# Suyashagarw/StreamOptima

Hardware: AMD Instinct MI355X
Metric: encoded Mpixels/sec at 1080p & 4K, 1/2/4/8 GPUs; PSNR delta vs reference (higher is better)
Workload: dtype u8

## Files before the change

### streamoptima_amd/csrc/so_block.h

```cpp
#pragma once
#include "so_common.h"
#include "so_dct.h"

namespace so {

SO_DEV void wave_sync() {
    __builtin_amdgcn_fence(__ATOMIC_RELEASE, "wavefront");
    __builtin_amdgcn_wave_barrier();
    __builtin_amdgcn_fence(__ATOMIC_ACQUIRE, "wavefront");
}

SO_DEV int scan_index(int n, int i, int j) {
    const int k = i + j;
    const int before = (k < n) ? (k * (k + 1)) / 2 : n * n - ((2 * n - 1 - k) * (2 * n - k)) / 2;
    const int first_i = (k < n) ? 0 : k - n + 1;
    return before + (i - first_i);
}

template <int G>
SO_DEV int group_sum(int v) {
#pragma unroll
    for (int m = G / 2; m >= 1; m >>= 1) v += __shfl_xor(v, m, 64);
    return v;
}

template <int NB>
SO_DEV void fetch_row(const uint8_t* __restrict__ f, int W, int H, int px, int py, bool fast, int* out) {
    if (fast) {
        const uint8_t* p = f + (size_t)py * W + px;
        const uintptr_t a = reinterpret_cast<uintptr_t>(p);
        const uint32_t* q = reinterpret_cast<const uint32_t*>(a & ~(uintptr_t)3);
        const uint32_t sh = (uint32_t)(a & 3);
        uint32_t w[NB / 4 + 1];
#pragma unroll
        for (int k = 0; k <= NB / 4; ++k) w[k] = q[k];
#pragma unroll
        for (int k = 0; k < NB / 4; ++k) {
            uint32_t v = __builtin_amdgcn_alignbyte(w[k + 1], w[k], sh);
            out[4 * k + 0] = v & 255;
            out[4 * k + 1] = (v >> 8) & 255;
            out[4 * k + 2] = (v >> 16) & 255;
            out[4 * k + 3] = v >> 24;
        }
    } else {
#pragma unroll
        for (int k = 0; k < NB; ++k) {
            const int xx = px + k;
            out[k] = (py >= 0 && py < H && xx >= 0 && xx < W) ? f[(size_t)py * W + xx] : 0;
        }
    }
}

template <int NB>
SO_DEV void fetch_row_fme(const uint8_t* __restrict__ planes, size_t pstride, int W, int H, int px, int py, int row,
                          int ext, int lim, int* out) {
    const int W2 = 2 * W - 1, H2 = 2 * H - 1;
    if (0 <= px && px < W2 - NB && 0 <= py && py < H2 - NB) {
        if (0 <= px + ext && px + ext < W2 - lim && 0 <= py + ext && py + ext < H2 - lim) {
            const uint8_t* pl = planes + (size_t)(2 * (py & 1) + (px & 1)) * pstride;
            fetch_row<NB>(pl, W, H, px >> 1, (py >> 1) + row, true, out);
        } else {
#pragma unroll
            for (int k = 0; k < NB; ++k) out[k] = 128;
        }
    } else {
        const int Y = py + row;
#pragma unroll
        for (int k = 0; k < NB; ++k) {
            const int X = px + k;
            out[k] = (Y >= 0 && Y < H2 && X >= 0 && X < W2)
                         ? planes[(size_t)(2 * (Y & 1) + (X & 1)) * pstride + (size_t)(Y >> 1) * W + (X >> 1)]
                         : 0;
        }
    }
}

template <int NB>
SO_DEV void load_cur_row(const uint8_t* __restrict__ f, int W, int x, int y, int* out) {
    const uint8_t* p = f + (size_t)y * W + x;
    if constexpr (NB == 16) {
        uint4 v = *reinterpret_cast<const uint4*>(p);
        uint32_t w[4] = {v.x, v.y, v.z, v.w};
#pragma unroll
        for (int k = 0; k < 16; ++k) out[k] = (w[k >> 2] >> (8 * (k & 3))) & 255;
    } else {
        uint2 v = *reinterpret_cast<const uint2*>(p);
        uint32_t w[2] = {v.x, v.y};
#pragma unroll
        for (int k = 0; k < 8; ++k) out[k] = (w[k >> 2] >> (8 * (k & 3))) & 255;
    }
}

template <int NB>
SO_DEV void store_row_u8(uint8_t* __restrict__ f, int W, int x, int y, const int* v) {
    uint32_t w[NB / 4];
#pragma unroll
    for (int k = 0; k < NB / 4; ++k)
        w[k] = (uint32_t)(v[4 * k] & 255) | ((uint32_t)(v[4 * k + 1] & 255) << 8) |
               ((uint32_t)(v[4 * k + 2] & 255) << 16) | ((uint32_t)(v[4 * k + 3] & 255) << 24);
    uint8_t* p = f + (size_t)y * W + x;
    if constexpr (NB == 16) *reinterpret_cast<uint4*>(p) = make_uint4(w[0], w[1], w[2], w[3]);
    else *reinterpret_cast<uint2*>(p) = make_uint2(w[0], w[1]);
}

template <int NB>
SO_DEV void store_row_i16(int16_t* __restrict__ p, const int* v) {
    uint32_t w[NB / 2];
#pragma unroll
    for (int k = 0; k < NB / 2; ++k) w[k] = (uint32_t)(uint16_t)v[2 * k] | ((uint32_t)(uint16_t)v[2 * k + 1] << 16);
    if constexpr (NB == 16) {
        reinterpret_cast<uint4*>(p)[0] = make_uint4(w[0], w[1], w[2], w[3]);
        reinterpret_cast<uint4*>(p)[1] = make_uint4(w[4], w[5], w[6], w[7]);
    } else {
        reinterpret_cast<uint4*>(p)[0] = make_uint4(w[0], w[1], w[2], w[3]);
    }
}

template <int NB>
SO_DEV void load_row_i16(const int16_t* __restrict__ p, int* v) {
    uint32_t w[NB / 2];
    if constexpr (NB == 16) {
        uint4 a = reinterpret_cast<const uint4*>(p)[0], b = reinterpret_cast<const uint4*>(p)[1];
        w[0] = a.x; w[1] = a.y; w[2] = a.z; w[3] = a.w; w[4] = b.x; w[5] = b.y; w[6] = b.z; w[7] = b.w;
    } else {
        uint4 a = reinterpret_cast<const uint4*>(p)[0];
        w[0] = a.x; w[1] = a.y; w[2] = a.z; w[3] = a.w;
    }
#pragma unroll
    for (int k = 0; k < NB / 2; ++k) {
        v[2 * k] = (int)(int16_t)(w[k] & 0xFFFF);
        v[2 * k + 1] = (int)(int16_t)(w[k] >> 16);
    }
}

template <int N, bool INVERSE, class T, class TWt = typename dct::Rfft<N>::TW>
SO_DEV void xform2d_rows(double* lds, int l, const T* in_row, double* out_row, const TWt& tw = TWt{}) {
    constexpr int P = N + 1;
    double v[N];
    if constexpr (N == 16 && __is_same(T, int)) {
        int* const li = reinterpret_cast<int*>(lds);
#pragma unroll
        for (int c = 0; c < N; ++c) li[l * P + c] = in_row[c];
        wave_sync();
        int x[N];
#pragma unroll
        for (int r = 0; r < N; ++r) x[r] = li[r * P + l];
        wave_sync();
        if constexpr (INVERSE) dct::dct3_16_i(x, v, tw); else dct::dct2_16_i(x, v, tw);
    } else {
#pragma unroll
        for (int c = 0; c < N; ++c) lds[l * P + c] = (double)in_row[c];
        wave_sync();
#pragma unroll
        for (int r = 0; r < N; ++r) v[r] = lds[r * P + l];
        if constexpr (INVERSE) dct::dct3<N>(v, tw); else dct::dct2<N>(v, tw);
    }
#pragma unroll
    for (int r = 0; r < N; ++r) lds[r * P + l] = v[r];
    wave_sync();
#pragma unroll
    for (int c = 0; c < N; ++c) v[c] = lds[l * P + c];
    if constexpr (INVERSE) dct::dct3<N>(v, tw); else dct::dct2<N>(v, tw);
#pragma unroll
    for (int c = 0; c < N; ++c) out_row[c] = v[c];
    wave_sync();
}

template <bool INVERSE, class TWt>
SO_DEV void xform2d_rows_dw(double* lds, int l, const int* in_row, double* out_row, const TWt& tw) {
    constexpr int N = 16, P = N + 1;
    typedef __attribute__((address_space(3))) uint32_t* lds_u32p;
    lds_u32p rowp = (lds_u32p)(reinterpret_cast<uint32_t*>(lds) + l * P);
    lds_u32p colp = (lds_u32p)(reinterpret_cast<uint32_t*>(lds) + l);
    asm volatile("" : "+v"(rowp), "+v"(colp));
    double v[N];
    {
#pragma unroll
        for (int c = 0; c < N; ++c) rowp[c] = (uint32_t)in_row[c];
        wave_sync();
        int x[N];
#pragma unroll
        for (int r = 0; r < N; ++r) x[r] = (int)colp[r * P];
        wave_sync();
        if constexpr (INVERSE) dct::dct3_16_i(x, v, tw); else dct::dct2_16_i(x, v, tw);
    }
    uint32_t lo[N];
#pragma unroll
    for (int r = 0; r < N; ++r) colp[r * P] = (uint32_t)__builtin_bit_cast(uint64_t, v[r]);
    wave_sync();
#pragma unroll
    for (int c = 0; c < N; ++c) lo[c] = rowp[c];
    wave_sync();
#pragma unroll
    for (int r = 0; r < N; ++r) colp[r * P] = (uint32_t)(__builtin_bit_cast(uint64_t, v[r]) >> 32);
    wave_sync();
#pragma unroll
    for (int c = 0; c < N; ++c)
        v[c] = __builtin_bit_cast(double, ((uint64_t)rowp[c] << 32) | (uint64_t)lo[c]);
    if constexpr (INVERSE) dct::dct3<N>(v, tw); else dct::dct2<N>(v, tw);
#pragma unroll
    for (int c = 0; c < N; ++c) out_row[c] = v[c];
    wave_sync();
}

template <bool INVERSE, bool DW, class FT>
SO_DEV void xform2d_fast(double* lds, int l, const int* in_row, double (&v)[16], const FT& ft) {
    constexpr int N = 16, P = N + 1;
    typedef __attribute__((address_space(3))) uint32_t* lds_u32p;
    lds_u32p rowp = (lds_u32p)(reinterpret_cast<uint32_t*>(lds) + l * P);
    lds_u32p colp = (lds_u32p)(reinterpret_cast<uint32_t*>(lds) + l);
    if constexpr (DW) asm volatile("" : "+v"(rowp), "+v"(colp));
    {
#pragma unroll
        for (int c = 0; c < N; ++c) rowp[c] = (uint32_t)in_row[c];
        wave_sync();
        int x[N];
#pragma unroll
        for (int r = 0; r < N; ++r) x[r] = (int)colp[r * P];
        wave_sync();
        if constexpr (INVERSE) {
#pragma unroll
            for (int r = 0; r < N; ++r) v[r] = (double)x[r];
            dct::dct3_16_fast(v, ft);
        } else {
            dct::dct2_16_fast_i(x, v, ft);
        }
    }
    if constexpr (DW) {
        uint32_t lo[N];
#pragma unroll
        for (int r = 0; r < N; ++r) colp[r * P] = (uint32_t)__builtin_bit_cast(uint64_t, v[r]);
        wave_sync();
#pragma unroll
        for (int c = 0; c < N; ++c) lo[c] = rowp[c];
        wave_sync();
#pragma unroll
        for (int r = 0; r < N; ++r) colp[r * P] = (uint32_t)(__builtin_bit_cast(uint64_t, v[r]) >> 32);
        wave_sync();
#pragma unroll
        for (int c = 0; c < N; ++c) v[c] = __builtin_bit_cast(double, ((uint64_t)rowp[c] << 32) | (uint64_t)lo[c]);
    } else {
#pragma unroll
        for (int r = 0; r < N; ++r) lds[r * P + l] = v[r];
        wave_sync();
#pragma unroll
        for (int c = 0; c < N; ++c) v[c] = lds[l * P + c];
    }
    if constexpr (INVERSE) dct::dct3_16_fast(v, ft); else dct::dct2_16_fast(v, ft);
    wave_sync();
}

template <class TWt>
SO_DEV void xform2d_fwd_i_half(double* lds, int l, const int* in_row, double* out_row, const TWt& tw) {
    constexpr int N = 16, PI = N + 1, P = 9;
    const int hl = l >> 3, cl = l & 7;
    double v[N];
    {
        int* const li = reinterpret_cast<int*>(lds);
#pragma unroll
        for (int c = 0; c < N; ++c) li[l * PI + c] = in_row[c];
        wave_sync();
        int x[N];
#pragma unroll
        for (int r = 0; r < N; ++r) x[r] = li[r * PI + l];
        wave_sync();
        dct::dct2_16_i(x, v, tw);
    }
#pragma unroll
    for (int h = 0; h < 2; ++h) {
        if (hl == h) {
#pragma unroll
            for (int r = 0; r < N; ++r) lds[r * P + cl] = v[r];
        }
        wave_sync();
#pragma unroll
        for (int c = 0; c < 8; ++c) out_row[8 * h + c] = lds[l * P + c];
        wave_sync();
    }
    dct::dct2<N>(out_row, tw);
}

template <bool INVERSE, class T>
SO_DEV void xform2d_rows_half(double* lds, int l, const T* in_row, double* out_row) {
    constexpr int N = 16, P = 9;
    const int hl = l >> 3, cl = l & 7;
    double v[N];
#pragma unroll
    for (int h = 0; h < 2; ++h) {
#pragma unroll
        for (int c = 0; c < 8; ++c) lds[l * P + c] = (double)in_row[8 * h + c];
        wave_sync();
        if (hl == h) {
#pragma unroll
            for (int r = 0; r < N; ++r) v[r] = lds[r * P + cl];
        }
        wave_sync();
    }
    if constexpr (INVERSE) dct::dct3<N>(v); else dct::dct2<N>(v);
#pragma unroll
    for (int h = 0; h < 2; ++h) {
        if (hl == h) {
#pragma unroll
            for (int r = 0; r < N; ++r) lds[r * P + cl] = v[r];
        }
        wave_sync();
#pragma unroll
        for (int c = 0; c < 8; ++c) out_row[8 * h + c] = lds[l * P + c];
        wave_sync();
    }
    if constexpr (INVERSE) dct::dct3<N>(out_row); else dct::dct2<N>(out_row);
}

template <bool INVERSE, class T, class TWt = dct::TW8>
SO_DEV void xform2d_sub(double* lds, int l, const T (&in)[2][8], double (&out)[2][8], const TWt& tw = TWt{}) {
    const int j = l >> 2, r0 = l & 3;
    double* s = lds + j * 72;
    if constexpr (__is_same(T, int)) {
        int* const si = reinterpret_cast<int*>(s);
#pragma unroll
        for (int h = 0; h < 2; ++h)
#pragma unroll
            for (int c = 0; c < 8; ++c) si[(r0 + 4 * h) * 9 + c] = in[h][c];
        wave_sync();
        int x[2][8];
#pragma unroll
        for (int h = 0; h < 2; ++h)
#pragma unroll
            for (int r = 0; r < 8; ++r) x[h][r] = si[r * 9 + r0 + 4 * h];
        wave_sync();
#pragma unroll
        for (int h = 0; h < 2; ++h) {
            double v[8];
            if constexpr (INVERSE) dct::dct3_8_i(x[h], v, tw); else dct::dct2_8_i(x[h], v, tw);
#pragma unroll
            for (int r = 0; r < 8; ++r) s[r * 9 + r0 + 4 * h] = v[r];
        }
    } else {
#pragma unroll
        for (int h = 0; h < 2; ++h)
#pragma unroll
            for (int c = 0; c < 8; ++c) s[(r0 + 4 * h) * 9 + c] = (double)in[h][c];
        wave_sync();
#pragma unroll
        for (int h = 0; h < 2; ++h) {
            double v[8];
            const int col = r0 + 4 * h;
#pragma unroll
            for (int r = 0; r < 8; ++r) v[r] = s[r * 9 + col];
            if constexpr (INVERSE) dct::dct3<8>(v, tw); else dct::dct2<8>(v, tw);
#pragma unroll
            for (int r = 0; r < 8; ++r) s[r * 9 + col] = v[r];
        }
    }
    wave_sync();
#pragma unroll
    for (int h = 0; h < 2; ++h) {
        double v[8];
        const int row = r0 + 4 * h;
#pragma unroll
        for (int c = 0; c < 8; ++c) v[c] = s[row * 9 + c];
        if constexpr (INVERSE) dct::dct3<8>(v, tw); else dct::dct2<8>(v, tw);
#pragma unroll
        for (int c = 0; c < 8; ++c) out[h][c] = v[c];
    }
    wave_sync();
}

template <int N>
SO_DEV void quant_row(const int* tc, int row, int qp, int* q) {
#pragma unroll
    for (int c = 0; c < N; ++c) q[c] = quant_rne(tc[c], q_exp(row, c, N, qp));
}

template <int N>
SO_DEV void dequant_row(const int* q, int row, int qp, int* d) {
#pragma unroll
    for (int c = 0; c < N; ++c) d[c] = q[c] * (1 << q_exp(row, c, N, qp));
}

template <int N>
SO_DEV int q_exp_fast(int row, int c, int qp) {
    const int s = row + c - (N - 2);
    return qp + (s < 0 ? 0 : (s > 2 ? 2 : s));
}

template <int N>
SO_DEV void quant_row_d(const double* tcr, int row, int qp, double* qd, int* q) {
#pragma unroll
    for (int c = 0; c < N; ++c) {
        qd[c] = __builtin_rint(__builtin_amdgcn_ldexp(tcr[c], -q_exp_fast<N>(row, c, qp)));
        q[c] = (int)qd[c];
    }
}

template <int N>
SO_DEV void dequant_row_d(const double* qd, int row, int qp, double* dq) {
#pragma unroll
    for (int c = 0; c < N; ++c) dq[c] = __builtin_amdgcn_ldexp(qd[c], q_exp_fast<N>(row, c, qp));
}

template <int N>
SO_DEV void quant_row_i(const int* tc, int row, int qp, int* q) {
#pragma unroll
    for (int c = 0; c < N; ++c)
        q[c] = (int)__builtin_rint(__builtin_amdgcn_ldexp((double)tc[c], -q_exp_fast<N>(row, c, qp)));
}

template <int N>
SO_DEV void dequant_row_i(const int* q, int row, int qp, double* dq) {
#pragma unroll
    for (int c = 0; c < N; ++c) dq[c] = __builtin_amdgcn_ldexp((double)q[c], q_exp_fast<N>(row, c, qp));
}

SO_DEV int quant_rne_i(int tc, int k) {
    const int bias = k > 0 ? ((1 << k) >> 1) - 1 + ((tc >> k) & 1) : 0;
    return (tc + bias) >> k;
}
template <int N>
SO_DEV void quant_row_int(const int* tc, int row, int qp, int* q) {
#pragma unroll
    for (int c = 0; c < N; ++c) q[c] = quant_rne_i(tc[c], q_exp_fast<N>(row, c, qp));
}

template <int N>
SO_DEV void dequant_row_int(const int* q, int row, int qp, int* dq) {
#pragma unroll
    for (int c = 0; c < N; ++c) dq[c] = (int)((uint32_t)q[c] << q_exp_fast<N>(row, c, qp));
}

template <int N>
SO_DEV int block_tokens(uint8_t* flags, int l, const int* q) {
    (void)flags;
    uint32_t m = 0;
#pragma unroll
    for (int c = 0; c < N; ++c) m |= (q[c] != 0 ? 1u : 0u) << c;
    const uint32_t mn = (uint32_t)__builtin_amdgcn_update_dpp(0, (int)m, 0x101, 0xF, 0xF, false);
    uint32_t m0, mlast;
    if constexpr (N == 16) {
        m0 = (uint32_t)__builtin_amdgcn_update_dpp(0, (int)m, 0x150, 0xF, 0xF, false);
        mlast = (uint32_t)__builtin_amdgcn_update_dpp(0, (int)m, 0x150 + N - 1, 0xF, 0xF, false);
    } else {
        const int base = (threadIdx.x & 63) & ~(N - 1);
        m0 = (uint32_t)__shfl((int)m, base, 64);
        mlast = (uint32_t)__shfl((int)m, base + N - 1, 64);
    }
    constexpr uint32_t kInner = ((1u << N) - 1) & ~1u;
    int tr = 0;
    if (l <= N - 2) {
        tr += __builtin_popcount((m ^ (mn << 1)) & kInner);
        tr += (int)((m & 1u) ^ ((m0 >> (l + 1)) & 1u));
    }
    if (l >= 1) tr += (int)(((mlast >> (l - 1)) & 1u) ^ ((m >> (N - 1)) & 1u));
    return group_sum<N>(__builtin_popcount(m) + tr) + 1;
}

SO_DEV int sub_tokens(uint8_t* flags, int l, const int (&q)[2][8]) {
    const int j = l >> 2, r0 = l & 3;
    uint8_t* s = flags + j * 64;
#pragma unroll
    for (int h = 0; h < 2; ++h)
#pragma unroll
        for (int c = 0; c < 8; ++c) s[scan_index(8, r0 + 4 * h, c)] = q[h][c] != 0;
    wave_sync();
    int nnz = 0, tr = 0;
    const int base = r0 * 16;
    int prev = s[base == 0 ? 0 : base - 1];
#pragma unroll
    for (int k = 0; k < 16; ++k) {
        const int f = s[base + k];
        nnz += f;
        tr += (f != prev);
        prev = f;
    }
    wave_sync();
    return group_sum<16>(nnz + tr) + 4;
}

SO_DEV int sub_tokens_reg(int l, const int (&q)[2][8]) {
    const int r0 = l & 3;
    uint32_t m0 = 0, m1 = 0;
#pragma unroll
    for (int c = 0; c < 8; ++c) {
        m0 |= (q[0][c] != 0 ? 1u : 0u) << c;
        m1 |= (q[1][c] != 0 ? 1u : 0u) << c;
    }
    uint32_t lo = m0 << (8 * r0), hi = m1 << (8 * r0);
    lo |= (uint32_t)__builtin_amdgcn_update_dpp(0, (int)lo, 0xB1, 0xF, 0xF, false);
    hi |= (uint32_t)__builtin_amdgcn_update_dpp(0, (int)hi, 0xB1, 0xF, 0xF, false);
    lo |= (uint32_t)__builtin_amdgcn_update_dpp(0, (int)lo, 0x4E, 0xF, 0xF, false);
    hi |= (uint32_t)__builtin_amdgcn_update_dpp(0, (int)hi, 0x4E, 0xF, 0xF, false);
    const uint32_t n0 = r0 < 3 ? (lo >> (8 * r0 + 8)) & 255u : hi & 255u;
    const uint32_t n1 = r0 < 3 ? (hi >> (8 * r0 + 8)) & 255u : 0u;
    const uint32_t M0 = lo & 255u, M7 = hi >> 24;
    int tr = __builtin_popcount((m0 ^ (n0 << 1)) & 0xFEu) + (int)((m0 & 1u) ^ ((M0 >> (r0 + 1)) & 1u)) +
             (int)(((M7 >> (r0 + 3)) & 1u) ^ (m1 >> 7));
    if (r0 < 3) tr += __builtin_popcount((m1 ^ (n1 << 1)) & 0xFEu) + (int)((m1 & 1u) ^ ((M0 >> (r0 + 5)) & 1u));
    if (r0 >= 1) tr += (int)(((M7 >> (r0 - 1)) & 1u) ^ (m0 >> 7));
    return group_sum<16>(__builtin_popcount(m0) + __builtin_popcount(m1) + tr) + 4;
}

SO_DEV double rd_cost(double lam, int bits, double mae) {
    const double lb = lam * (double)bits;
    return lb + mae;
}

}
```

### streamoptima_amd/csrc/so_me.hip

```cpp
#include <stdlib.h>
#include <string.h>

#include <array>
#include <cstring>
#include <map>
#include <mutex>
#include <type_traits>
#include <utility>

#include "so_block.h"
#include "so_common.h"
#include "so_dpp.h"
#include "so_run.h"

namespace so {

SO_DEV uint64_t me_key(uint32_t sad, uint32_t l1, uint32_t ref, uint32_t scan) {
    return ((uint64_t)sad << 32) | ((uint64_t)l1 << 24) | ((uint64_t)ref << 16) | (uint64_t)scan;
}
constexpr uint64_t kNoKey = ~0ull;
constexpr uint32_t kDenseSadOps = 1152u * 256u;
#define SO_OPS_ADD(p, v) do { if (L.count_ops) atomicAdd((p), (v)); } while (0)

SO_DEV void decode_key(uint64_t k, int sr, int32_t* out) {
// ... 1220 lines not shown
                        sad = __builtin_amdgcn_sad_u8(cr[rr][0], __builtin_amdgcn_alignbyte(q1, q0, sh), sad);
                        sad = __builtin_amdgcn_sad_u8(cr[rr][1], __builtin_amdgcn_alignbyte(q2, q1, sh), sad);
                        sad = __builtin_amdgcn_sad_u8(cr[rr][2], __builtin_amdgcn_alignbyte(q3, q2, sh), sad);
                        sad = __builtin_amdgcn_sad_u8(cr[rr][3], __builtin_amdgcn_alignbyte(q4, q3, sh), sad);
                    }
                    sad = quad_sum_u32(sad);
                    const int dx = dxi - 16, dy = di - 16;
                    const uint64_t key = me_key(sad, (uint32_t)((dx < 0 ? -dx : dx) + (dy < 0 ? -dy : dy)),
                                                (uint32_t)r, (uint32_t)cand);
                    best = (act && key < best) ? key : best;
                }
            }
            best = wave_min_u64_dpp(best);
            if (lane == 0 && best < keys[u]) keys[u] = best;
        }
    }
    SO_MARK(search_end);
    __syncthreads();
}

__global__ void __launch_bounds__(Sea2Geo::NTHREADS) __attribute__((amdgpu_waves_per_eu(kSea2Wpe)))
me_sea2_kernel(const uint8_t* __restrict__ cur, RefSet refs, int nref, int H, int W, int by0, int by1,
               int32_t* __restrict__ out_best, int probe) {
    using G = Sea2Geo;
    constexpr int SR = G::SR, TBX = G::TBX, TBY = G::TBY, RP = G::RP, B4P = G::B4P;
    __shared__ uint32_t win[G::WR * RP + 4];
    __shared__ uint32_t b4w[(G::B4RS * B4P + 4) / 4];
    __shared__ uint32_t curt[G::TPY * G::CPD];
    __shared__ uint32_t a4[G::NBLK * 4];
    __shared__ uint16_t list[G::NW * G::CAPL];
    __shared__ uint32_t lcount[G::NW];
    __shared__ unsigned long long keys[G::NBLK];
    __shared__ uint32_t st[3];
    const Sea2Lds L{win, b4w, curt, a4, list, lcount, keys, st};
    SO_STAMP_REC_SET(g_sea_stamps ? g_sea_stamps + (size_t)blockIdx.x * 12 : nullptr);
    sea2_tile<Sea2Geo>(L, blockIdx.x, cur, refs, nref, H, W, by0, by1, probe);

    const int tid = threadIdx.x;
    const int nbx = W / 16;
    const int tiles_x = (nbx + TBX - 1) / TBX;
    const int bx0 = (blockIdx.x % tiles_x) * TBX, byt0 = by0 + (blockIdx.x / tiles_x) * TBY;
    SO_SEA_STAMP(5, __builtin_amdgcn_s_memtime());
    for (int i = tid; i < G::NBLK; i += G::NTHREADS) {
        const int gbx = bx0 + i % TBX, gby = byt0 + i / TBX;
        if (gbx >= nbx || gby >= by1) continue;
        decode_key(keys[i], SR, out_best + ((size_t)(gby - by0) * nbx + gbx) * 4);
    }
#ifdef SO_STAMPS
    if (tid == 0) {
        uint32_t hw, xcc;
        asm volatile("s_getreg_b32 %0, hwreg(HW_REG_HW_ID)" : "=s"(hw));
        asm volatile("s_getreg_b32 %0, hwreg(HW_REG_XCC_ID)" : "=s"(xcc));
        SO_SEA_STAMP(6, __builtin_amdgcn_s_memtime());
        SO_SEA_STAMP(7, __builtin_amdgcn_s_memrealtime());
        SO_SEA_STAMP(8, ((unsigned long long)xcc << 32) | hw);
        SO_SEA_STAMP(9, ((unsigned long long)st[0] << 32) | st[1]);
    }
#endif
}

constexpr int kTqScratch = 16 * 17;
constexpr int kTqScratchHalf = 16 * 9;
constexpr int kTqScratchDw = 16 * 17 / 2;
template <class G, bool HALFTQ>
constexpr int tq_scratch() {
    return HALFTQ ? kTqScratchHalf : (G::TQDW ? kTqScratchDw : kTqScratch);
}
#ifndef SO_FWD_MFMA
#define SO_FWD_MFMA 0
#endif
template <class G, bool HALFTQ = false>
struct PTileGeo {
    static constexpr int B4 = (G::B4RS * G::B4P + 4) / 4;
    static constexpr int LIST = G::NW * G::CAPL / 2;
    static constexpr int TQD = G::NBLK * tq_scratch<G, HALFTQ>();
    static constexpr int U64 = ((B4 + LIST + 1) / 2 > TQD) ? (B4 + LIST + 1) / 2 : TQD;
};
constexpr int kTqScratchVbs = 288;
template <class G>
struct PTileGeoVbs {
    static constexpr int TQD = G::NBLK * kTqScratchVbs;
    static constexpr int U64 = ((PTileGeo<G>::B4 + PTileGeo<G>::LIST + 1) / 2 > TQD)
                                   ? (PTileGeo<G>::B4 + PTileGeo<G>::LIST + 1) / 2 : TQD;
};

template <int RP>
SO_DEV void win_row16(const uint32_t* win, int row, int col, uint32_t (&w)[4]) {
    lds_vu32p p = (lds_vu32p)(win + row * RP + (col >> 2));
    const uint32_t sh = (uint32_t)(col & 3);
    const uint32_t q0 = p[0], q1 = p[1], q2 = p[2], q3 = p[3], q4 = p[4];
    w[0] = __builtin_amdgcn_alignbyte(q1, q0, sh);
    w[1] = __builtin_amdgcn_alignbyte(q2, q1, sh);
    w[2] = __builtin_amdgcn_alignbyte(q3, q2, sh);
    w[3] = __builtin_amdgcn_alignbyte(q4, q3, sh);
}

typedef uint32_t so_v4u __attribute__((ext_vector_type(4)));

struct MeRec {
    uint16_t v[4];
    SO_DEV int operator[](int k) const { return k < 3 ? (int)(int16_t)v[k] : (v[3] == 0xFFFFu ? -1 : (int)v[3]); }
    SO_DEV void set(const int32_t (&r)[4]) {
#pragma unroll
        for (int k = 0; k < 4; ++k) v[k] = (uint16_t)r[k];
    }
};

template <class G, bool VBS = false, bool HALFTQ = false>
struct PTileLds {
    static constexpr int NU = G::NBLK * (VBS ? 5 : 1);
    uint32_t win[G::WR * G::RP + 4];
    uint32_t curt[G::TPY * G::CPD];
    uint32_t a4[G::NBLK * 4];
    uint32_t lcount[G::NW];
    unsigned long long keys[NU];
    uint32_t st[3];
    MeRec mer[NU];
    int32_t msum[G::TBY];
    uint32_t fwd_flags;
    alignas(16) double un[VBS ? PTileGeoVbs<G>::U64 : PTileGeo<G, HALFTQ>::U64];
    uint8_t vsp[VBS ? G::NBLK : 1];
};

struct PHalo {
    uint8_t* up;
    uint8_t* dn;
    int up_end, dn_begin;
};

#ifndef SO_TQ_FAST
#define SO_TQ_FAST 1
#endif
#define SO_TQ_FT() dct::ft16_table()
template <class G, bool SC1, bool HALO = false, bool TOK = false, bool HALFTQ = false, bool ZSKIP = false,
          bool FAST = false>
SO_DEV void tq16_exact(PTileLds<G, false, HALFTQ>& S, int g, int l, double* scratch, int bx0, int byt0, int nbx, int by0, int by1,
                       int W, int qp_rd, const int32_t* __restrict__ qp_row, const int32_t* __restrict__ qp_map,
                       const PFrameOut& o, const PHalo& hl = PHalo{}, bool qs = false) {
    constexpr int SR = G::SR, TBX = G::TBX;
    const int bxl = g % TBX, byl = g / TBX;
    const int gbx = bx0 + bxl, gby = byt0 + byl;
    if (gbx < nbx && gby < by1) {
        size_t b = (size_t)(gby - by0) * nbx + gbx;
        int x = gbx * 16, y = gby * 16;
        const int qpr = qp_map ? qp_map[(size_t)gby * nbx + gbx] : (qp_row ? qp_row[gby] : qp_rd);
        const int dx = S.mer[g][0], dy = S.mer[g][1], rf = S.mer[g][2], sad = S.mer[g][3];
        const int prow = byl * 16 + SR + dy + l, pcol = bxl * 16 + SR + dx;
        const uint32_t* crow = S.curt + (byl * 16 + l) * G::CPD + bxl * 4;
        double* dl = scratch;
        constexpr double kRne = 0x1.8p52;
        const auto derive = [&]() {
            if constexpr (FAST) {
                asm volatile("" : "+v"(g), "+v"(l));
                const int gbx2 = bx0 + g % TBX, gby2 = byt0 + g / TBX;
                b = (size_t)(gby2 - by0) * nbx + gbx2;
                x = gbx2 * 16;
                y = gby2 * 16;
                dl = S.un + g * tq_scratch<G, HALFTQ>();
            }
        };
        const auto rows_of = [&](int g2, int l2, int& prow2, int& pcol2, const uint32_t*& crow2) {
            asm volatile("" : "+v"(g2), "+v"(l2));
            const int bxl2 = g2 % TBX, byl2 = g2 / TBX;
            lds_vu32p mp = (lds_vu32p)reinterpret_cast<const uint32_t*>(&S.mer[g2]);
            const uint32_t w0 = mp[0];
            prow2 = byl2 * 16 + SR + ((int)w0 >> 16) + l2;
            pcol2 = bxl2 * 16 + SR + (int)(int16_t)(w0 & 0xFFFFu);
            crow2 = S.curt + (byl2 * 16 + l2) * G::CPD + bxl2 * 4;
        };
        int q[16];
        if (qs) {
            const so_v4u* qr = reinterpret_cast<const so_v4u*>(reinterpret_cast<const int16_t*>(dl) + l * 16);
#pragma unroll
            for (int h = 0; h < 2; ++h) {
                const so_v4u v = qr[h];
#pragma unroll
                for (int e = 0; e < 4; ++e) {
                    q[8 * h + 2 * e] = (int)(int16_t)(v[e] & 0xFFFFu);
                    q[8 * h + 2 * e + 1] = (int)v[e] >> 16;
                }
            }
        } else {
            SO_MARK(tq_residual);
            int res[16];
            const auto load_res = [&](int prow_, int pcol_, const uint32_t* crow_) {
                uint32_t pw[4];
                win_row16<G::RP>(S.win, prow_, pcol_, pw);
#pragma unroll
                for (int k = 0; k < 4; ++k) {
                    const uint32_t cw = crow_[k];
#pragma unroll
                    for (int e = 0; e < 4; ++e)
                        res[4 * k + e] = (int)((cw >> (8 * e)) & 255) - (int)((pw[k] >> (8 * e)) & 255);
                }
            };
            load_res(prow, pcol, crow);
            double tcr[16];
            SO_MARK(tq_fwd);
            static_assert(!HALFTQ || TOK, "the half scratch carries the forward transform only");
            static_assert(!FAST || (!HALFTQ && !TOK && !HALO), "the fast transforms: the plain run only");
            const int sc_hi2 = (1023 - 2 - qpr) << 20;
            const auto quant_fma = [&](bool certify) -> bool {
                int sc_hi = (1023 - qpr - (l == 15 ? 1 : 0)) << 20;
                bool flag = false;
#pragma unroll
                for (int c0 = 0; c0 < 16; c0 += 4) {
                    uint64_t nm[4], any = 0;
#pragma unroll
                    for (int j = 0; j < 4; ++j) {
                        const int c = c0 + j;
                        const double sc = __builtin_bit_cast(double, (uint64_t)(uint32_t)sc_hi << 32);
                        const double r = __builtin_rint(tcr[c]);
                        q[c] = (int)(uint32_t)__builtin_bit_cast(uint64_t, __builtin_fma(r, sc, kRne));
                        if (certify) {
                            nm[j] = __builtin_amdgcn_ballot_w64(__builtin_fabs(tcr[c] - r) >= 0.5 - dct::kFastDeltaFwd);
                            any |= nm[j];
                        }
                        if (c < 15) sc_hi = __builtin_amdgcn_update_dpp(sc_hi2, sc_hi, 0x101, 0xF, 0xF, false);
                    }
#ifdef SO_TQ_CENSUS_NO_NEAR
                    any = 0;
#endif
                    if (certify && any != 0) {
                        SO_MARK(tq_fwd_near);
#pragma unroll
                        for (int j = 0; j < 4; ++j) {
                            if (nm[j] != 0) {
                                const int c = c0 + j;
                                const double sc = __builtin_bit_cast(
                                    double, (uint64_t)(uint32_t)((1023 - q_exp_fast<16>(l, c, qpr)) << 20) << 32);
                                const double r = __builtin_rint(tcr[c]), d = tcr[c] - r;
                                const double r2 = r + __builtin_copysign(1.0, d);
                                const int q2 = (int)(uint32_t)__builtin_bit_cast(uint64_t, __builtin_fma(r2, sc, kRne));
                                flag |= __builtin_fabs(d) >= 0.5 - dct::kFastDeltaFwd && q2 != q[c];
                            }
                        }
                        SO_MARK(tq_quant);
                    }
                }
                return certify && __builtin_amdgcn_ballot_w64(flag) != 0;
            };
            if constexpr (FAST) {
                xform2d_fast<false, G::TQDW>(dl, l, res, tcr, SO_TQ_FT());
                asm volatile("" : "+v"(tcr[0]), "+v"(tcr[1]), "+v"(tcr[2]), "+v"(tcr[3]), "+v"(tcr[4]), "+v"(tcr[5]),
                             "+v"(tcr[6]), "+v"(tcr[7]));
                asm volatile("" : "+v"(tcr[8]), "+v"(tcr[9]), "+v"(tcr[10]), "+v"(tcr[11]), "+v"(tcr[12]), "+v"(tcr[13]),
                             "+v"(tcr[14]), "+v"(tcr[15]));
                SO_MARK(tq_quant);
                if (quant_fma(true)) {
                    SO_MARK(tq_fwd_fallback);
                    const uint64_t act = __builtin_amdgcn_ballot_w64(true);
                    if ((int)(threadIdx.x & 63) == __builtin_ctzll(act)) atomicAdd(reinterpret_cast<uint32_t*>(&S.msum[0]), 1u);
                    int prow2, pcol2;
                    const uint32_t* crow2;
                    rows_of(g, l, prow2, pcol2, crow2);
                    load_res(prow2, pcol2, crow2);
                    if constexpr (G::TQDW)
                        xform2d_rows_dw<false>(dl, l, res, tcr, dct::tw16_table());
                    else
                        xform2d_rows<16, false>(dl, l, res, tcr, dct::tw16_table());
                    quant_fma(false);
                }
            } else {
            if constexpr (HALFTQ)
                xform2d_fwd_i_half(dl, l, res, tcr, dct::tw16_table());
            else if constexpr (G::TQDW)
                xform2d_rows_dw<false>(dl, l, res, tcr, dct::tw16_table());
            else
                xform2d_rows<16, false>(dl, l, res, tcr, dct::tw16_table());
            SO_MARK(tq_quant);
#pragma unroll
            for (int c = 0; c < 16; ++c)
                q[c] = (int)(uint32_t)__builtin_bit_cast(
                    uint64_t, __builtin_amdgcn_ldexp(__builtin_rint(tcr[c]), -q_exp_fast<16>(l, c, qpr)) + kRne);
            }
        }
        SO_MARK(tq_tokens);
        derive();
        const int tok = block_tokens<16>(nullptr, l, q);
        if constexpr (TOK) {
            if (l == 0) o.tokens[b] = tok;
            return;
        }
        SO_MARK(tq_qtc_store);
        store_row_i16<16>(o.qtc + b * 256 + l * 16, q);
        const auto finish = [&](const int (&rec)[16]) -> int {
            if constexpr (SC1) {
                so_v4u v;
#pragma unroll
                for (int k = 0; k < 4; ++k)
                    v[k] = (uint32_t)(rec[4 * k] & 255) | ((uint32_t)(rec[4 * k + 1] & 255) << 8) |
                           ((uint32_t)(rec[4 * k + 2] & 255) << 16) | ((uint32_t)(rec[4 * k + 3] & 255) << 24);
                uint8_t* rp = o.recon + (size_t)(y + l) * W + x;
                asm volatile("global_store_dwordx4 %0, %1, off sc1" ::"v"(rp), "v"(v) : "memory");
                if constexpr (HALO) {
                    if (hl.up && y + l < hl.up_end) {
                        uint8_t* q2 = hl.up + (size_t)(y + l) * W + x;
                        asm volatile("global_store_dwordx4 %0, %1, off sc0 sc1" ::"v"(q2), "v"(v) : "memory");
                    }
                    if (hl.dn && y + l >= hl.dn_begin) {
                        uint8_t* q2 = hl.dn + (size_t)(y + l) * W + x;
                        asm volatile("global_store_dwordx4 %0, %1, off sc0 sc1" ::"v"(q2), "v"(v) : "memory");
                    }
                }
            } else {
                store_row_u8<16>(o.recon, W, x, y + l, rec);
            }
            SO_MARK(tq_sse_records);
            int e2 = 0;
            if (o.sse) {
                const uint32_t* crow2 = crow;
                if constexpr (G::TQDW) {
                    int g2 = g, l2 = l;
                    asm volatile("" : "+v"(g2), "+v"(l2));
                    crow2 = S.curt + ((g2 / TBX) * 16 + l2) * G::CPD + (g2 % TBX) * 4;
                }
#pragma unroll
                for (int k = 0; k < 4; ++k) {
                    const uint32_t cw = crow2[k];
#pragma unroll
                    for (int e = 0; e < 4; ++e) {
                        const int d = (int)((cw >> (8 * e)) & 255) - (rec[4 * k + e] & 255);
                        e2 += d * d;
                    }
                }
                e2 = group_sum<16>(e2);
            }
            return e2;
        };
        const auto full_exact = [&](const int (&ql)[16]) -> int {
            int dq[16];
            double rd[16];
            dequant_row_int<16>(ql, l, qpr, dq);
            if constexpr (!FAST) SO_MARK(tq_inv);
            if constexpr (G::TQDW)
                xform2d_rows_dw<true>(dl, l, dq, rd, dct::tw16_table());
            else
                xform2d_rows<16, true>(dl, l, dq, rd, dct::tw16_table());
            if constexpr (!FAST) SO_MARK(tq_recon);
            derive();
            int rec[16];
            {
                int prow2 = prow, pcol2 = pcol;
                if constexpr (FAST) {
                    const uint32_t* crow2;
                    rows_of(g, l, prow2, pcol2, crow2);
                }
                uint32_t pw[4];
                win_row16<G::RP>(S.win, prow2, pcol2, pw);
#pragma unroll
                for (int c = 0; c < 16; ++c)
                    rec[c] = (int)((pw[c >> 2] >> (8 * (c & 3))) & 255) +
                             (int)(uint32_t)__builtin_bit_cast(uint64_t, rd[c] + kRne);
            }
            return finish(rec);
        };
        const auto full = [&]() -> int {
            if constexpr (FAST) {
                {
                    int dq[16], rec[16];
                    double rd[16];
                    {
                        int k = qpr + (l == 15 ? 1 : 0);
#pragma unroll
                        for (int c = 0; c < 16; ++c) {
                            dq[c] = (int)((uint32_t)q[c] << k);
                            if (c < 15) k = __builtin_amdgcn_update_dpp(qpr + 2, k, 0x101, 0xF, 0xF, false);
                        }
                    }
                    SO_MARK(tq_inv);
                    xform2d_fast<true, G::TQDW>(dl, l, dq, rd, SO_TQ_FT());
                    asm volatile("" : "+v"(rd[0]), "+v"(rd[1]), "+v"(rd[2]), "+v"(rd[3]), "+v"(rd[4]), "+v"(rd[5]),
                                 "+v"(rd[6]), "+v"(rd[7]));
                    asm volatile("" : "+v"(rd[8]), "+v"(rd[9]), "+v"(rd[10]), "+v"(rd[11]), "+v"(rd[12]), "+v"(rd[13]),
                                 "+v"(rd[14]), "+v"(rd[15]));
                    SO_MARK(tq_recon);
                    derive();
                    constexpr double kFix = 0x1.8p28 + 0.5;
                    uint32_t mn = 0xFFFFFFFFu;
                    {
                        int prow2, pcol2;
                        const uint32_t* crow2;
                        rows_of(g, l, prow2, pcol2, crow2);
                        uint32_t pw[4];
                        win_row16<G::RP>(S.win, prow2, pcol2, pw);
#pragma unroll
                        for (int c = 0; c < 16; ++c) {
                            const uint32_t gfix = (uint32_t)__builtin_bit_cast(uint64_t, rd[c] + kFix);
                            rec[c] = (int)(((((pw[c >> 2] >> (8 * (c & 3))) & 255u) << 24) + gfix) >> 24);
                            const uint32_t t = (gfix + 2u) << 8;
                            mn = t < mn ? t : mn;
                        }
                    }
                    if (__builtin_amdgcn_ballot_w64(mn <= (4u << 8)) == 0) return finish(rec);
                }
                SO_MARK(tq_inv_fallback);
                const uint64_t act = __builtin_amdgcn_ballot_w64(true);
                if ((int)(threadIdx.x & 63) == __builtin_ctzll(act)) atomicAdd(reinterpret_cast<uint32_t*>(&S.msum[1]), 1u);
                int qf[16];
                load_row_i16<16>(o.qtc + b * 256 + l * 16, qf);
                return full_exact(qf);
            } else {
                return full_exact(q);
            }
        };
        int sse;
        if constexpr (ZSKIP) {
            if (__builtin_amdgcn_ballot_w64(tok != 1) == 0) {
                int rec[16];
                uint32_t pw[4];
                win_row16<G::RP>(S.win, prow, pcol, pw);
#pragma unroll
                for (int c = 0; c < 16; ++c) rec[c] = (int)((pw[c >> 2] >> (8 * (c & 3))) & 255);
                sse = finish(rec);
            } else {
                sse = full();
            }
        } else {
            sse = full();
        }
        int mdx = dx, mdy = dy, mrf = rf, msad = sad;
        if constexpr (G::TQDW) {
            int g2 = g;
            asm volatile("" : "+v"(g2));
            lds_vu32p mp = (lds_vu32p)reinterpret_cast<const uint32_t*>(&S.mer[g2]);
            const uint32_t w0 = mp[0], w1 = mp[1];
            mdx = (int)(int16_t)(w0 & 0xFFFFu);
            mdy = (int)w0 >> 16;
            mrf = (int)(int16_t)(w1 & 0xFFFFu);
            msad = (w1 >> 16) == 0xFFFFu ? -1 : (int)(w1 >> 16);
        }
        if (l < 12) o.mv[b * 12 + l] = (int16_t)(l == 0 ? mdx : l == 1 ? mdy : l == 2 ? mrf : 0);
        if (l == 0) {
            o.split[b] = 0;
            o.tokens[b] = tok;
            o.mae[b] = msad;
            if (o.sse) o.sse[b] = sse;
        }
    }
}

__constant__ float kDctCos32[17] = {
    0x1.6a09e6p-2f, 0x1.684b9cp-2f, 0x1.63150cp-2f, 0x1.5a730cp-2f, 0x1.4e7aeap-2f, 0x1.3f4a24p-2f,
    0x1.2d062ep-2f, 0x1.17dc14p-2f, 0x1.000000p-2f, 0x1.cb598cp-3f, 0x1.92469cp-3f, 0x1.5553e4p-3f,
    0x1.1517a8p-3f, 0x1.a4608ap-4f, 0x1.1a855ep-4f, 0x1.1be352p-5f, 0.0f};

SO_DEV float dct16_f32(int u, int r) {
    if (u == 0) return 0.25f;
    const int j = ((2 * r + 1) * u) & 63;
    const int m = j <= 32 ? j : 64 - j;
    return m <= 16 ? kDctCos32[m] : -kDctCos32[32 - m];
}

typedef float so_v4f __attribute__((ext_vector_type(4)));
constexpr float kFwdBound = 2.6e-7f;

template <class G, bool HALFTQ>
SO_DEV void fwd_mfma(PTileLds<G, false, HALFTQ>& S, int g, int ln, const float (&cs)[4], int bx0, int byt0, int nbx, int by1,
                     int qp_rd, const int32_t* __restrict__ qp_row, const int32_t* __restrict__ qp_map) {
    constexpr int SR = G::SR, TBX = G::TBX;
    const int bxl = g % TBX, byl = g / TBX;
    const int gbx = bx0 + bxl, gby = byt0 + byl;
    if (gbx >= nbx || gby >= by1) return;
    const int qpr = qp_map ? qp_map[(size_t)gby * nbx + gbx] : (qp_row ? qp_row[gby] : qp_rd);
    const int r = ln & 15, c4 = ln >> 4;
    const int dx = S.mer[g][0], dy = S.mer[g][1];
    const uint32_t cw = S.curt[(byl * 16 + r) * G::CPD + bxl * 4 + c4];
    const uint32_t pw = win_u32<G::RP>(S.win, byl * 16 + SR + dy + r, bxl * 16 + SR + dx + 4 * c4);
    float a[4];
    uint32_t sab = 0;
#pragma unroll
    for (int s = 0; s < 4; ++s) {
        const int d = (int)((cw >> (8 * s)) & 255) - (int)((pw >> (8 * s)) & 255);
        a[s] = (float)d;
        sab += (uint32_t)(d < 0 ? -d : d);
    }
    sab = wave_sum_u32(sab);
    so_v4f y = {0.f, 0.f, 0.f, 0.f}, z = {0.f, 0.f, 0.f, 0.f};
#pragma unroll
    for (int s = 0; s < 4; ++s) y = __builtin_amdgcn_mfma_f32_16x16x4f32(a[s], cs[s], y, 0, 0, 0);
#pragma unroll
    for (int s = 0; s < 4; ++s) z = __builtin_amdgcn_mfma_f32_16x16x4f32(cs[s], y[s], z, 0, 0, 0);
    const float delta = __builtin_fmaf((float)sab, kFwdBound, 0x1p-20f);
    bool near = qpr < 1;
    int16_t* qd = reinterpret_cast<int16_t*>(S.un + g * tq_scratch<G, HALFTQ>());
#pragma unroll
    for (int i = 0; i < 4; ++i) {
        const int u = 4 * c4 + i, k = q_exp_fast<16>(u, r, qpr);
        const float zi = z[i];
        const float mid = __builtin_amdgcn_ldexpf(__builtin_floorf(__builtin_amdgcn_ldexpf(zi, -k)) + 0.5f, k);
        near |= __builtin_fabsf(__builtin_fabsf(zi - mid) - 0.5f) <= delta;
        qd[u * 16 + r] = (int16_t)(int)__builtin_rintf(__builtin_amdgcn_ldexpf(__builtin_rintf(zi), -k));
    }
#ifdef SO_FWD_FORCE
    near = SO_FWD_FORCE;
#endif
    if (__builtin_amdgcn_ballot_w64(near) != 0 && ln == 0) atomicOr(&S.fwd_flags, 1u << g);
}

template <int NBLK>
SO_DEV int fwd_order(uint32_t m, int p) {
    const int nf = __builtin_popcount(m);
    uint32_t s = p < nf ? m : (~m & ((1u << NBLK) - 1u));
    for (int t = p < nf ? p : p - nf; t > 0; --t) s &= s - 1u;
    return __builtin_ctz(s);
}

template <int RP>
SO_DEV void win_row8(const uint32_t* win, int row, int col, uint32_t (&w)[2]) {
    lds_vu32p p = (lds_vu32p)(win + row * RP + (col >> 2));
    const uint32_t sh = (uint32_t)(col & 3);
    const uint32_t q0 = p[0], q1 = p[1], q2 = p[2];
    w[0] = __builtin_amdgcn_alignbyte(q1, q0, sh);
    w[1] = __builtin_amdgcn_alignbyte(q2, q1, sh);
}

template <bool SC1, bool HALO>
SO_DEV void store_rec_row(const PFrameOut& o, const PHalo& hl, int W, int x, int yy, const int* rec, int n) {
    uint8_t* rp = o.recon + (size_t)yy * W + x;
    if (n == 16) {
        so_v4u v;
#pragma unroll
        for (int k = 0; k < 4; ++k)
            v[k] = (uint32_t)(rec[4 * k] & 255) | ((uint32_t)(rec[4 * k + 1] & 255) << 8) |
                   ((uint32_t)(rec[4 * k + 2] & 255) << 16) | ((uint32_t)(rec[4 * k + 3] & 255) << 24);
        if constexpr (SC1) {
            asm volatile("global_store_dwordx4 %0, %1, off sc1" ::"v"(rp), "v"(v) : "memory");
            if constexpr (HALO) {
                if (hl.up && yy < hl.up_end) {
                    uint8_t* q = hl.up + (size_t)yy * W + x;
                    asm volatile("global_store_dwordx4 %0, %1, off sc0 sc1" ::"v"(q), "v"(v) : "memory");
                }
                if (hl.dn && yy >= hl.dn_begin) {
                    uint8_t* q = hl.dn + (size_t)yy * W + x;
                    asm volatile("global_store_dwordx4 %0, %1, off sc0 sc1" ::"v"(q), "v"(v) : "memory");
                }
            }
        } else {
            *reinterpret_cast<so_v4u*>(rp) = v;
        }
    } else {
        typedef uint32_t so_v2u __attribute__((ext_vector_type(2)));
        so_v2u v;
#pragma unroll
        for (int k = 0; k < 2; ++k)
            v[k] = (uint32_t)(rec[4 * k] & 255) | ((uint32_t)(rec[4 * k + 1] & 255) << 8) |
                   ((uint32_t)(rec[4 * k + 2] & 255) << 16) | ((uint32_t)(rec[4 * k + 3] & 255) << 24);
        if constexpr (SC1) {
            asm volatile("global_store_dwordx2 %0, %1, off sc1" ::"v"(rp), "v"(v) : "memory");
            if constexpr (HALO) {
                if (hl.up && yy < hl.up_end) {
                    uint8_t* q = hl.up + (size_t)yy * W + x;
                    asm volatile("global_store_dwordx2 %0, %1, off sc0 sc1" ::"v"(q), "v"(v) : "memory");
                }
                if (hl.dn && yy >= hl.dn_begin) {
                    uint8_t* q = hl.dn + (size_t)yy * W + x;
                    asm volatile("global_store_dwordx2 %0, %1, off sc0 sc1" ::"v"(q), "v"(v) : "memory");
                }
            }
        } else {
            *reinterpret_cast<so_v2u*>(rp) = v;
        }
    }
}

template <int N>
SO_DEV void pack_i16(const int* v, uint32_t* p) {
// ... 1522 lines not shown
```

Measured before the change: 179,300.

## Keep reconstructed rows packed as bytes and use SDWA adds, udot4 SSE and DPP row sums

In the FAST transform-quantize path, reconstructed pixels now stay packed four per dword. Byte-wise SDWA adds apply the residual to the prediction, replacing per-pixel unpack, shift and repack. The SSE is computed with udot4 (c²+r²−2cr) on the packed words, and row reductions for SSE and token counts use a DPP row sum instead of shuffle-xor trees. Tile index division is done as unsigned. This cuts VALU instruction count in the reconstruction and distortion stage, at the cost of inline assembly that relies on the byte arithmetic not overflowing, which depends on the existing fallback check.

```diff
diff --git a/streamoptima_amd/csrc/so_block.h b/streamoptima_amd/csrc/so_block.h
--- a/streamoptima_amd/csrc/so_block.h
+++ b/streamoptima_amd/csrc/so_block.h
@@ -1,6 +1,7 @@
 #pragma once
 #include "so_common.h"
 #include "so_dct.h"
+#include "so_dpp.h"
 
 namespace so {
 
@@ -133,6 +134,32 @@
     }
 }
 
+#define SO_RP(k, e, g)                                                                              \
+    "v_add_u32_sdwa %" #k ", %" #k ", %" #g " dst_sel:BYTE_" #e " dst_unused:UNUSED_PRESERVE src0_sel:BYTE_" #e \
+    " src1_sel:BYTE_3\n\t"
+SO_DEV void recon_row_bytes(uint32_t (&pw)[4], const uint32_t (&g)[16]) {
+    asm(SO_RP(0, 0, 4) SO_RP(1, 0, 8) SO_RP(2, 0, 12) SO_RP(3, 0, 16)
+        SO_RP(0, 1, 5) SO_RP(1, 1, 9) SO_RP(2, 1, 13) SO_RP(3, 1, 17)
+        SO_RP(0, 2, 6) SO_RP(1, 2, 10) SO_RP(2, 2, 14) SO_RP(3, 2, 18)
+        SO_RP(0, 3, 7) SO_RP(1, 3, 11) SO_RP(2, 3, 15) SO_RP(3, 3, 19) "s_nop 0"
+        : "+v"(pw[0]), "+v"(pw[1]), "+v"(pw[2]), "+v"(pw[3])
+        : "v"(g[0]), "v"(g[1]), "v"(g[2]), "v"(g[3]), "v"(g[4]), "v"(g[5]), "v"(g[6]), "v"(g[7]), "v"(g[8]),
+          "v"(g[9]), "v"(g[10]), "v"(g[11]), "v"(g[12]), "v"(g[13]), "v"(g[14]), "v"(g[15]));
+}
+#undef SO_RP
+
+SO_DEV int sse_row_packed(const uint32_t* c, const uint32_t (&r)[4]) {
+    uint32_t sq = 0, cr = 0;
+#pragma unroll
+    for (int k = 0; k < 4; ++k) {
+        const uint32_t cw = c[k];
+        sq = __builtin_amdgcn_udot4(cw, cw, sq, false);
+        sq = __builtin_amdgcn_udot4(r[k], r[k], sq, false);
+        cr = __builtin_amdgcn_udot4(cw, r[k], cr, false);
+    }
+    return (int)(sq - 2u * cr);
+}
+
 template <int N, bool INVERSE, class T, class TWt = typename dct::Rfft<N>::TW>
 SO_DEV void xform2d_rows(double* lds, int l, const T* in_row, double* out_row, const TWt& tw = TWt{}) {
     constexpr int P = N + 1;
@@ -428,7 +455,7 @@
     for (int c = 0; c < N; ++c) dq[c] = (int)((uint32_t)q[c] << q_exp_fast<N>(row, c, qp));
 }
 
-template <int N>
+template <int N, bool ROWSUM = false>
 SO_DEV int block_tokens(uint8_t* flags, int l, const int* q) {
     (void)flags;
     uint32_t m = 0;
@@ -451,7 +478,12 @@
         tr += (int)((m & 1u) ^ ((m0 >> (l + 1)) & 1u));
     }
     if (l >= 1) tr += (int)(((mlast >> (l - 1)) & 1u) ^ ((m >> (N - 1)) & 1u));
-    return group_sum<N>(__builtin_popcount(m) + tr) + 1;
+    if constexpr (ROWSUM) {
+        static_assert(N == 16, "a DPP row is 16 lanes");
+        return (int)row_sum_u32((uint32_t)(__builtin_popcount(m) + tr)) + 1;
+    } else {
+        return group_sum<N>(__builtin_popcount(m) + tr) + 1;
+    }
 }
 
 SO_DEV int sub_tokens(uint8_t* flags, int l, const int (&q)[2][8]) {
diff --git a/streamoptima_amd/csrc/so_me.hip b/streamoptima_amd/csrc/so_me.hip
--- a/streamoptima_amd/csrc/so_me.hip
+++ b/streamoptima_amd/csrc/so_me.hip
@@ -1396,7 +1396,7 @@
         const auto derive = [&]() {
             if constexpr (FAST) {
                 asm volatile("" : "+v"(g), "+v"(l));
-                const int gbx2 = bx0 + g % TBX, gby2 = byt0 + g / TBX;
+                const int gbx2 = bx0 + (int)((uint32_t)g % TBX), gby2 = byt0 + (int)((uint32_t)g / TBX);
                 b = (size_t)(gby2 - by0) * nbx + gbx2;
                 x = gbx2 * 16;
                 y = gby2 * 16;
@@ -1405,7 +1405,7 @@
         };
         const auto rows_of = [&](int g2, int l2, int& prow2, int& pcol2, const uint32_t*& crow2) {
             asm volatile("" : "+v"(g2), "+v"(l2));
-            const int bxl2 = g2 % TBX, byl2 = g2 / TBX;
+            const int bxl2 = (int)((uint32_t)g2 % TBX), byl2 = (int)((uint32_t)g2 / TBX);
             lds_vu32p mp = (lds_vu32p)reinterpret_cast<const uint32_t*>(&S.mer[g2]);
             const uint32_t w0 = mp[0];
             prow2 = byl2 * 16 + SR + ((int)w0 >> 16) + l2;
@@ -1521,20 +1521,25 @@
         }
         SO_MARK(tq_tokens);
         derive();
-        const int tok = block_tokens<16>(nullptr, l, q);
+        const int tok = block_tokens<16, FAST>(nullptr, l, q);
         if constexpr (TOK) {
             if (l == 0) o.tokens[b] = tok;
             return;
         }
         SO_MARK(tq_qtc_store);
         store_row_i16<16>(o.qtc + b * 256 + l * 16, q);
-        const auto finish = [&](const int (&rec)[16]) -> int {
+        static_assert(!FAST || SC1, "the packed row goes to the write-through store");
+        const auto finish = [&](const auto& rec) -> int {
             if constexpr (SC1) {
                 so_v4u v;
-#pragma unroll
-                for (int k = 0; k < 4; ++k)
-                    v[k] = (uint32_t)(rec[4 * k] & 255) | ((uint32_t)(rec[4 * k + 1] & 255) << 8) |
-                           ((uint32_t)(rec[4 * k + 2] & 255) << 16) | ((uint32_t)(rec[4 * k + 3] & 255) << 24);
+                if constexpr (FAST) {
+                    v = so_v4u{rec[0], rec[1], rec[2], rec[3]};
+                } else {
+#pragma unroll
+                    for (int k = 0; k < 4; ++k)
+                        v[k] = (uint32_t)(rec[4 * k] & 255) | ((uint32_t)(rec[4 * k + 1] & 255) << 8) |
+                               ((uint32_t)(rec[4 * k + 2] & 255) << 16) | ((uint32_t)(rec[4 * k + 3] & 255) << 24);
+                }
                 uint8_t* rp = o.recon + (size_t)(y + l) * W + x;
                 asm volatile("global_store_dwordx4 %0, %1, off sc1" ::"v"(rp), "v"(v) : "memory");
                 if constexpr (HALO) {
@@ -1559,16 +1564,20 @@
                     asm volatile("" : "+v"(g2), "+v"(l2));
                     crow2 = S.curt + ((g2 / TBX) * 16 + l2) * G::CPD + (g2 % TBX) * 4;
                 }
-#pragma unroll
-                for (int k = 0; k < 4; ++k) {
-                    const uint32_t cw = crow2[k];
-#pragma unroll
-                    for (int e = 0; e < 4; ++e) {
-                        const int d = (int)((cw >> (8 * e)) & 255) - (rec[4 * k + e] & 255);
-                        e2 += d * d;
+                if constexpr (FAST) {
+                    e2 = sse_row_packed(crow2, rec);
+                } else {
+#pragma unroll
+                    for (int k = 0; k < 4; ++k) {
+                        const uint32_t cw = crow2[k];
+#pragma unroll
+                        for (int e = 0; e < 4; ++e) {
+                            const int d = (int)((cw >> (8 * e)) & 255) - (rec[4 * k + e] & 255);
+                            e2 += d * d;
+                        }
                     }
                 }
-                e2 = group_sum<16>(e2);
+                if constexpr (FAST) e2 = (int)row_sum_u32((uint32_t)e2); else e2 = group_sum<16>(e2);
             }
             return e2;
         };
@@ -1597,12 +1606,21 @@
                     rec[c] = (int)((pw[c >> 2] >> (8 * (c & 3))) & 255) +
                              (int)(uint32_t)__builtin_bit_cast(uint64_t, rd[c] + kRne);
             }
-            return finish(rec);
+            if constexpr (FAST) {
+                uint32_t v[4];
+#pragma unroll
+                for (int k = 0; k < 4; ++k)
+                    v[k] = (uint32_t)(rec[4 * k] & 255) | ((uint32_t)(rec[4 * k + 1] & 255) << 8) |
+                           ((uint32_t)(rec[4 * k + 2] & 255) << 16) | ((uint32_t)(rec[4 * k + 3] & 255) << 24);
+                return finish(v);
+            } else {
+                return finish(rec);
+            }
         };
         const auto full = [&]() -> int {
             if constexpr (FAST) {
                 {
-                    int dq[16], rec[16];
+                    int dq[16];
                     double rd[16];
                     {
                         int k = qpr + (l == 15 ? 1 : 0);
@@ -1622,21 +1640,22 @@
                     derive();
                     constexpr double kFix = 0x1.8p28 + 0.5;
                     uint32_t mn = 0xFFFFFFFFu;
+                    uint32_t pw[4];
                     {
                         int prow2, pcol2;
                         const uint32_t* crow2;
                         rows_of(g, l, prow2, pcol2, crow2);
-                        uint32_t pw[4];
                         win_row16<G::RP>(S.win, prow2, pcol2, pw);
+                        uint32_t gfix[16];
 #pragma unroll
                         for (int c = 0; c < 16; ++c) {
-                            const uint32_t gfix = (uint32_t)__builtin_bit_cast(uint64_t, rd[c] + kFix);
-                            rec[c] = (int)(((((pw[c >> 2] >> (8 * (c & 3))) & 255u) << 24) + gfix) >> 24);
-                            const uint32_t t = (gfix + 2u) << 8;
+                            gfix[c] = (uint32_t)__builtin_bit_cast(uint64_t, rd[c] + kFix);
+                            const uint32_t t = (gfix[c] + 2u) << 8;
                             mn = t < mn ? t : mn;
                         }
+                        recon_row_bytes(pw, gfix);
                     }
-                    if (__builtin_amdgcn_ballot_w64(mn <= (4u << 8)) == 0) return finish(rec);
+                    if (__builtin_amdgcn_ballot_w64(mn <= (4u << 8)) == 0) return finish(pw);
                 }
                 SO_MARK(tq_inv_fallback);
                 const uint64_t act = __builtin_amdgcn_ballot_w64(true);
@@ -1651,12 +1670,16 @@
         int sse;
         if constexpr (ZSKIP) {
             if (__builtin_amdgcn_ballot_w64(tok != 1) == 0) {
-                int rec[16];
                 uint32_t pw[4];
                 win_row16<G::RP>(S.win, prow, pcol, pw);
-#pragma unroll
-                for (int c = 0; c < 16; ++c) rec[c] = (int)((pw[c >> 2] >> (8 * (c & 3))) & 255);
-                sse = finish(rec);
+                if constexpr (FAST) {
+                    sse = finish(pw);
+                } else {
+                    int rec[16];
+#pragma unroll
+                    for (int c = 0; c < 16; ++c) rec[c] = (int)((pw[c >> 2] >> (8 * (c & 3))) & 255);
+                    sse = finish(rec);
+                }
             } else {
                 sse = full();
             }
```

Result: faster. 184,200, median of 6 (+2.8%).
